# jgrodzki/radix_sort

Hardware: AMD Instinct MI355X
Metric: Gkeys/sec (u64) (higher is better)
Workload: dtype u64

## Files before the change

### radix_sort_amd/csrc/rsx_small_kernel.hpp

```cpp
#pragma once
#include "rsx_device.hpp"

namespace rsx {

struct SmallArgs {
    const void* src;
    void* data;
    uint32_t n;
    uint32_t passes;
    uint32_t rank_atomic;
    uint32_t map_load;
    uint32_t map_store;
    DigitSpec spec[16];
    KeyXform xf;
    const uint32_t* top_tot;
    uint32_t cap;
    uint32_t no_skip;
    uint32_t group_shift;
    uint32_t key_offset, key_bytes;
    uint32_t* hint;
};

struct PassPlan {
    uint32_t first, end;
    uint32_t mask[8];
    uint32_t low[8];
    __device__ __forceinline__ void set_masks(const uint32_t key_offset, const uint32_t key_bytes) {
#pragma unroll
        for (int w = 0; w < 8; ++w) {
            uint32_t m = 0, l = 0;
#pragma unroll
            for (uint32_t b = 0; b < 4; ++b) {
                const uint32_t byte = 4u * (uint32_t)w + b;
                if (byte >= key_offset + first && byte < key_offset + key_bytes) m |= 0xFFu << (8u * b);
                if (byte >= key_offset && byte < key_offset + first) l |= 0xFFu << (8u * b);
            }
            mask[w] = m;
            low[w] = l;
        }
    }
};

#ifndef RSX_MEND_SLACK
#define RSX_MEND_SLACK 6u
#endif
__device__ __forceinline__ uint32_t first_digit_for(const uint32_t m, const uint32_t variable_bits, const uint32_t end) {
    const uint32_t lg = m <= 1u ? 0u : 32u - (uint32_t)__builtin_clz(m - 1u);
    const uint32_t need = 2u * lg > RSX_MEND_SLACK ? 2u * lg - RSX_MEND_SLACK : 0u;
    uint32_t first = variable_bits > need ? (variable_bits - need) >> 3 : 0u;
    if (first + 1u > end) first = end != 0u ? end - 1u : 0u;
    return first;
}

template <int ES>
struct WaveCnt {
    static constexpr bool HALF = false;
    using T = typename std::conditional<HALF, uint16_t, uint32_t>::type;
    static __device__ __forceinline__ void zero(T* my, uint32_t lane) {
        uint32_t* w = reinterpret_cast<uint32_t*>(my);
#pragma unroll
        for (int i = 0; i < (HALF ? 2 : 4); ++i) w[i * WAVE + lane] = 0;
    }
    static __device__ __forceinline__ uint32_t add_rtn(T* my, uint32_t d, uint32_t v) {
        if constexpr (HALF) {
            const uint32_t sh = (d & 1u) * 16u;
            return (atomicAdd(reinterpret_cast<uint32_t*>(my) + (d >> 1), v << sh) >> sh) & 0xFFFFu;
        } else {
            return atomicAdd(&my[d], v);
        }
    }
};
template <int ES, int KPT, int WG>
__host__ __device__ constexpr uint32_t cape() {
    constexpr uint32_t slots = (uint32_t)WG * KPT;
    constexpr uint32_t room = ((163840u - 1024u - (uint32_t)(WG / WAVE) * RADIX * (uint32_t)sizeof(typename WaveCnt<ES>::T) - 64u - 3u * RADIX * 4u) / (uint32_t)ES) & ~3u;
    return slots < room ? slots : room;
}

template <int ES, int KPT, int WG>
__device__ __forceinline__ void local_load(const SmallArgs& a, const Elem<ES>* __restrict__ src, const uint32_t n, Elem<ES> (&e)[KPT]) {
    const uint32_t tid = threadIdx.x, lane = tid & 63u, wave = tid >> 6;
    const uint32_t kp = (n + WG - 1) / WG;
    const uint32_t seg = wave * (WAVE * kp) + lane;
#pragma unroll
    for (int j = 0; j < KPT; ++j) {
        e[j] = Elem<ES>{};
        if ((uint32_t)j < kp) {
            const uint32_t p = seg + (uint32_t)j * WAVE;
            if (p < n) {
                e[j] = src[p];
                if (a.map_load) key_map<ES, false>(e[j], a.xf);
            }
        }
    }
}

template <int ES, int KPT, int WG>
__device__ __forceinline__ void local_passes(const SmallArgs& a, Elem<ES> (&e)[KPT], const uint32_t n, unsigned char* smem,
                                             const uint32_t first = 0, const uint32_t end = ~0u) {
    const uint32_t stop = end == ~0u ? a.passes : end;
    constexpr int NWAVE = WG / WAVE;
    using E = Elem<ES>;
    E* s_elems = reinterpret_cast<E*>(smem);
    using C = WaveCnt<ES>;
    typename C::T* s_cnt = reinterpret_cast<typename C::T*>(smem + (size_t)cape<ES, KPT, WG>() * sizeof(E));
    uint32_t* s_misc = reinterpret_cast<uint32_t*>(s_cnt + NWAVE * RADIX);
    const uint32_t tid = threadIdx.x, lane = tid & 63u, wave = tid >> 6;
    const uint32_t kp = (n + WG - 1) / WG;
    const uint32_t seg = wave * (WAVE * kp) + lane;
    typename C::T* my = s_cnt + wave * RADIX;
    for (uint32_t pass = first; pass < stop; ++pass) {
        const DigitSpec spec = a.spec[pass];
        C::zero(my, lane);
        auto digit_of = [&](int j) -> uint32_t {
            return (seg + (uint32_t)j * WAVE >= n) ? 255u : elem_digit<ES, false>(e[j], spec);
        };
        uint32_t rk[KPT];
#pragma unroll
        for (int j = 0; j < KPT; ++j) {
            rk[j] = 0;
            if ((uint32_t)j < kp) {
                const uint32_t d = digit_of(j);
                if (a.rank_atomic) {
                    rk[j] = C::add_rtn(my, d, 1u);
                } else {
                    const uint64_t m = match_digit(d);
                    const uint32_t below = mbcnt64(m);
                    const uint32_t seen = my[d];
                    if (below == 0) (void)C::add_rtn(my, d, (uint32_t)__popcll(m));
                    rk[j] = seen + below;
                }
            }
        }
        __syncthreads();
        uint32_t tcount = 0, incl = 0;
        if (tid < RADIX) {
#pragma unroll
            for (int w = 0; w < NWAVE; ++w) tcount += s_cnt[w * RADIX + tid];
            incl = wave_incl_scan<true>(tcount);
            if (lane == 63) s_misc[wave] = incl;
        }
        __syncthreads();
        if (tid < RADIX) {
            uint32_t run = incl - tcount;
            for (uint32_t w = 0; w < wave; ++w) run += s_misc[w];
#pragma unroll
            for (int w = 0; w < NWAVE; ++w) {
                const uint32_t c = s_cnt[w * RADIX + tid];
                s_cnt[w * RADIX + tid] = (typename C::T)run;
                run += c;
            }
        }
        __syncthreads();
#pragma unroll
        for (int j = 0; j < KPT; ++j)
            if ((uint32_t)j < kp) {
                if constexpr (cape<ES, KPT, WG>() < (uint32_t)WG * KPT) {
                    if (seg + (uint32_t)j * WAVE < n) s_elems[(uint32_t)my[digit_of(j)] + rk[j]] = e[j];
                } else {
                    s_elems[(uint32_t)my[digit_of(j)] + rk[j]] = e[j];
                }
            }
        __syncthreads();
        if (pass + 1 < stop) {
#pragma unroll
            for (int j = 0; j < KPT; ++j)
                if ((uint32_t)j < kp) e[j] = s_elems[seg + (uint32_t)j * WAVE];
        }
    }
}

template <int ES, int KPT, int WG>
__device__ __forceinline__ void local_store(const SmallArgs& a, Elem<ES>* __restrict__ dst, const uint32_t n, unsigned char* smem) {
    const Elem<ES>* s_elems = reinterpret_cast<const Elem<ES>*>(smem);
    for (uint32_t i = threadIdx.x; i < n; i += WG) {
        Elem<ES> x = s_elems[i];
        if (a.map_store) key_map<ES, true>(x, a.xf);
        dst[i] = x;
    }
}

template <int ES, int KPT, int WG>
__device__ __forceinline__ void local_sort(const SmallArgs& a, const Elem<ES>* __restrict__ src, Elem<ES>* __restrict__ dst,
                                           const uint32_t n, unsigned char* smem) {
    Elem<ES> e[KPT];
    local_load<ES, KPT, WG>(a, src, n, e);
    local_passes<ES, KPT, WG>(a, e, n, smem);
    local_store<ES, KPT, WG>(a, dst, n, smem);
}

template <int ES, int KPT, int WG, typename DigitFn>
__device__ __forceinline__ void stream_pass(const SmallArgs& a, const Elem<ES>* __restrict__ src, Elem<ES>* __restrict__ dst, const uint32_t m,
                                            unsigned char* smem, DigitFn digit, const bool map_back, uint32_t& bin_start, uint32_t& bin_count) {
    constexpr int NWAVE = WG / WAVE;
    constexpr uint32_t CH = cape<ES, KPT, WG>();
    using E = Elem<ES>;
    E* s_elems = reinterpret_cast<E*>(smem);
    using C = WaveCnt<ES>;
    typename C::T* s_cnt = reinterpret_cast<typename C::T*>(smem + (size_t)cape<ES, KPT, WG>() * sizeof(E));
    uint32_t* s_misc = reinterpret_cast<uint32_t*>(s_cnt + NWAVE * RADIX);
    uint32_t* s_gbase = s_misc + NWAVE;
    uint32_t* s_dstart = s_gbase + RADIX;
    uint32_t* s_dcount = s_dstart + RADIX;
    const uint32_t tid = threadIdx.x, lane = tid & 63u, wave = tid >> 6;
    typename C::T* my = s_cnt + wave * RADIX;
    if (tid < RADIX) s_gbase[tid] = 0;
    __syncthreads();
    for (uint32_t i = tid; i < m; i += WG) atomicAdd(&s_gbase[digit(src[i])], 1u);
    __syncthreads();
    if (tid < RADIX) {
        const uint32_t c = s_gbase[tid];
        const uint32_t incl = wave_incl_scan<true>(c);
        if (lane == 63) s_misc[wave] = incl;
        s_dcount[tid] = incl - c;
        bin_count = c;
    }
    __syncthreads();
    if (tid < RADIX) {
        uint32_t b = s_dcount[tid];
        for (uint32_t w = 0; w < wave; ++w) b += s_misc[w];
        s_gbase[tid] = b;
        bin_start = b;
    }
    __syncthreads();
    for (uint32_t c0 = 0; c0 < m; c0 += CH) {
        const uint32_t n = m - c0 < CH ? m - c0 : CH;
        const uint32_t kp = (n + WG - 1) / WG;
        const uint32_t seg = wave * (WAVE * kp) + lane;
        E e[KPT];
#pragma unroll
        for (int j = 0; j < KPT; ++j) {
            e[j] = E{};
            if ((uint32_t)j < kp) {
                const uint32_t p = seg + (uint32_t)j * WAVE;
                if (p < n) e[j] = src[c0 + p];
            }
        }
        C::zero(my, lane);
        auto digit_of = [&](int j) -> uint32_t { return (seg + (uint32_t)j * WAVE >= n) ? 255u : digit(e[j]); };
        uint32_t rk[KPT];
#pragma unroll
        for (int j = 0; j < KPT; ++j) {
            rk[j] = 0;
            if ((uint32_t)j < kp) {
                const uint32_t d = digit_of(j);
                const uint64_t mm = match_digit(d);
                const uint32_t below = mbcnt64(mm);
                const uint32_t seen = my[d];
                if (below == 0) (void)C::add_rtn(my, d, (uint32_t)__popcll(mm));
                rk[j] = seen + below;
            }
        }
        __syncthreads();
        uint32_t tcount = 0, incl = 0;
        if (tid < RADIX) {
#pragma unroll
            for (int w = 0; w < NWAVE; ++w) tcount += s_cnt[w * RADIX + tid];
            incl = wave_incl_scan<true>(tcount);
            if (lane == 63) s_misc[wave] = incl;
        }
        __syncthreads();
        if (tid < RADIX) {
            uint32_t run = incl - tcount;
            for (uint32_t w = 0; w < wave; ++w) run += s_misc[w];
            s_dstart[tid] = run;
            s_dcount[tid] = tid == RADIX - 1 ? tcount - (kp * WG - n) : tcount;
#pragma unroll
            for (int w = 0; w < NWAVE; ++w) {
                const uint32_t c = s_cnt[w * RADIX + tid];
                s_cnt[w * RADIX + tid] = (typename C::T)run;
                run += c;
            }
        }
        __syncthreads();
#pragma unroll
        for (int j = 0; j < KPT; ++j)
            if ((uint32_t)j < kp) {
                if constexpr (cape<ES, KPT, WG>() < (uint32_t)WG * KPT) {
                    if (seg + (uint32_t)j * WAVE < n) s_elems[(uint32_t)my[digit_of(j)] + rk[j]] = e[j];
                } else {
                    s_elems[(uint32_t)my[digit_of(j)] + rk[j]] = e[j];
                }
            }
        __syncthreads();
        for (uint32_t i = tid; i < n; i += WG) {
            E x = s_elems[i];
            const uint32_t d = digit(x);
            const uint32_t pos = s_gbase[d] + (i - s_dstart[d]);
            if (map_back) key_map<ES, true>(x, a.xf);
            dst[pos] = x;
        }
        __syncthreads();
        if (tid < RADIX) s_gbase[tid] += s_dcount[tid];
        __syncthreads();
    }
    __builtin_amdgcn_fence(__ATOMIC_RELEASE, "agent");
    __syncthreads();
    __builtin_amdgcn_fence(__ATOMIC_ACQUIRE, "agent");
}

template <int ES, int KPT, int WG>
__device__ void big_bucket_sort(const SmallArgs& a, Elem<ES>* buf0, Elem<ES>* buf1, const uint32_t m, unsigned char* smem) {
    using E = Elem<ES>;
    E* src = buf0;
    E* dst = buf1;
    for (uint32_t pass = 0; pass < a.passes; ++pass) {
        const DigitSpec spec = a.spec[pass];
        uint32_t bs = 0, bc = 0;
        stream_pass<ES, KPT, WG>(a, src, dst, m, smem, [&](const E& x) { return elem_digit<ES, false>(x, spec); },
                                 pass + 1 == a.passes && a.map_store != 0, bs, bc);
        E* t = src;
        src = dst;
        dst = t;
    }
}

#define RSX_B16_WAVES(WG) ((WG) >= 512 ? 4 : 3)
template <int ES>
__device__ __forceinline__ bool agree(const PassPlan& pp, const Elem<ES>& x, const Elem<ES>& y) {
    uint32_t diff = 0;
#pragma unroll
    for (int w = 0; w < ES / 4; ++w) diff |= (x.w[w] ^ y.w[w]) & pp.mask[w];
    return diff == 0;
}
constexpr uint32_t MEND_LIST = 192;
template <int ES, int KPT, int WG>
__device__ __forceinline__ uint32_t* mend_count(unsigned char* smem) {
    return reinterpret_cast<uint32_t*>(smem + (size_t)cape<ES, KPT, WG>() * sizeof(Elem<ES>));
}
template <int ES, int KPT, int WG>
__device__ __forceinline__ bool local_check(const PassPlan& pp, const uint32_t n, unsigned char* smem, Elem<ES> (&x)[KPT], uint32_t& ties) {
    using E = Elem<ES>;
    const E* s_elems = reinterpret_cast<const E*>(smem);
    ties = 0;
    if (threadIdx.x == 0) *mend_count<ES, KPT, WG>(smem) = 0;
#pragma unroll
    for (int j = 0; j < KPT; ++j) {
        const uint32_t i = (uint32_t)j * WG + threadIdx.x;
        x[j] = E{};
        if (i < n) {
            x[j] = s_elems[i];
            const E p = s_elems[i != 0 ? i - 1 : 0];
            uint32_t diff = 0;
#pragma unroll
            for (int w = 0; w < ES / 4; ++w) diff |= (x[j].w[w] ^ p.w[w]) & pp.mask[w];
            ties |= (diff == 0 && i != 0) ? 1u << j : 0u;
        }
    }
    uint32_t work = 0;
    for (uint32_t t = ties; t != 0; t &= t - 1u) {
        const uint32_t i = (uint32_t)__builtin_ctz(t) * WG + threadIdx.x;
        const E u = s_elems[i], v = s_elems[i - 1];
#pragma unroll
        for (int w = 0; w < ES / 4; ++w) work |= (u.w[w] ^ v.w[w]) & pp.low[w];
    }
    return __syncthreads_or(work != 0 ? 1 : 0) != 0;
}
#ifndef RSX_MEND_INLINE
#define RSX_MEND_INLINE __forceinline__
#endif
template <int ES>
struct MendMasks {
    uint32_t hi[ES / 4], lo[ES / 4];
};
template <int ES>
__device__ RSX_MEND_INLINE uint32_t mend_listed(Elem<ES>* s_elems, uint32_t* s_list, uint32_t* s_flag, const uint32_t n, const uint32_t wg,
                                                          uint32_t ties, const MendMasks<ES> mm) {
    using E = Elem<ES>;
    constexpr uint32_t MAX_RUN = 48;
    auto same = [&](const E& u, const E& v) {
        uint32_t diff = 0;
#pragma unroll
        for (int w = 0; w < ES / 4; ++w) diff |= (u.w[w] ^ v.w[w]) & mm.hi[w];
        return diff == 0;
    };
    auto less = [&](const E& u, const E& v) {
#pragma unroll
        for (int w = ES / 4 - 1; w >= 0; --w) {
            const uint32_t a = u.w[w] & mm.lo[w], b = v.w[w] & mm.lo[w];
            if (a != b) return a < b;
        }
        return false;
    };
    if (threadIdx.x == 0) *s_flag = 0;
    for (uint32_t j = 0; ties != 0; ++j, ties >>= 1) {
        if (!(ties & 1u)) continue;
        const uint32_t i = j * wg + threadIdx.x;
        if (i >= 2 && same(s_elems[i - 1], s_elems[i - 2])) continue;
        const uint32_t k = atomicAdd(&s_list[0], 1u);
        if (k < MEND_LIST) s_list[1 + k] = i - 1;
    }
    __syncthreads();
    const uint32_t heads = s_list[0];
    if (heads > MEND_LIST) return 0u;
    if (threadIdx.x < heads) {
        const uint32_t i = s_list[1 + threadIdx.x];
        uint32_t len = 2;
        while (i + len < n && len <= MAX_RUN && same(s_elems[i + len], s_elems[i])) ++len;
        if (len > MAX_RUN) {
            *s_flag = 1;
        } else {
            for (uint32_t k = 1; k < len; ++k) {
                const E y = s_elems[i + k];
                uint32_t j = k;
                while (j > 0 && less(y, s_elems[i + j - 1])) {
                    s_elems[i + j] = s_elems[i + j - 1];
                    --j;
                }
                s_elems[i + j] = y;
            }
        }
    }
    __syncthreads();
    return *s_flag == 0 ? 1u : 0u;
}
template <int ES, int KPT, int WG>
__device__ __forceinline__ bool local_mend_listed(const uint32_t n, unsigned char* smem, const PassPlan& pp, uint32_t* s_flag, const uint32_t ties) {
    static_assert((WG / WAVE) * RADIX >= MEND_LIST + 1, "the list lives in the wave counters");
    MendMasks<ES> mm;
#pragma unroll
    for (int w = 0; w < ES / 4; ++w) {
        mm.hi[w] = pp.mask[w];
        mm.lo[w] = pp.low[w];
    }
    return mend_listed<ES>(reinterpret_cast<Elem<ES>*>(smem), mend_count<ES, KPT, WG>(smem), s_flag, n, (uint32_t)WG, ties, mm) != 0;
}
template <int ES, int KPT, int WG>
__device__ __forceinline__ void local_store_regs(const SmallArgs& a, Elem<ES>* __restrict__ dst, const uint32_t n, Elem<ES> (&x)[KPT]) {
#pragma unroll
    for (int j = 0; j < KPT; ++j) {
        const uint32_t i = (uint32_t)j * WG + threadIdx.x;
        if (i < n) {
            if (a.map_store) key_map<ES, true>(x[j], a.xf);
            dst[i] = x[j];
        }
    }
}

template <int ES, int KPT, int WG>
__device__ __forceinline__ bool local_finish(const SmallArgs& a, Elem<ES>* __restrict__ dst, const uint32_t n, unsigned char* smem, const PassPlan& pp,
                                             uint32_t* s_flag) {
    Elem<ES> x[KPT];
    uint32_t ties;
    if (!local_check<ES, KPT, WG>(pp, n, smem, x, ties)) {
        local_store_regs<ES, KPT, WG>(a, dst, n, x);
        return true;
    }
    if (!local_mend_listed<ES, KPT, WG>(n, smem, pp, s_flag, ties)) return false;
    local_store<ES, KPT, WG>(a, dst, n, smem);
    return true;
}

template <int ES, int KPT, int WG>
__device__ __forceinline__ void local_sort_skip(const SmallArgs& a, const Elem<ES>* __restrict__ src, Elem<ES>* __restrict__ dst, const uint32_t n,
                                                unsigned char* smem, PassPlan& pp, uint32_t* s_flag) {
    using E = Elem<ES>;
    E e[KPT];
    local_load<ES, KPT, WG>(a, src, n, e);
    local_passes<ES, KPT, WG>(a, e, n, smem, pp.first, pp.end);
    if (pp.first == 0) {
        local_store<ES, KPT, WG>(a, dst, n, smem);
    } else if (!local_finish<ES, KPT, WG>(a, dst, n, smem, pp, s_flag)) {
        pp.first = 0;
        const uint32_t kp = (n + WG - 1) / WG, seg = (threadIdx.x >> 6) * (WAVE * kp) + (threadIdx.x & 63u);
#pragma unroll
        for (int j = 0; j < KPT; ++j)
            if ((uint32_t)j < kp) e[j] = reinterpret_cast<const E*>(smem)[seg + (uint32_t)j * WAVE];
        __syncthreads();
        local_passes<ES, KPT, WG>(a, e, n, smem, 0, pp.end);
        local_store<ES, KPT, WG>(a, dst, n, smem);
    }
}

template <int ES, int KPT>
__global__ __launch_bounds__(512) void rsx_small_sort_kernel(const SmallArgs a) {
    extern __shared__ __attribute__((aligned(16))) unsigned char smem[];
    local_sort<ES, KPT, 512>(a, static_cast<const Elem<ES>*>(a.src), static_cast<Elem<ES>*>(a.data), a.n, smem);
}

template <int ES, int KPT, int WG>
__global__ __launch_bounds__(WG) void rsx_bucket_sort_kernel(const SmallArgs a) {
    extern __shared__ __attribute__((aligned(16))) unsigned char smem[];
    uint64_t* s_red = reinterpret_cast<uint64_t*>(smem);
    const uint32_t tid = threadIdx.x, v = blockIdx.x;
    uint64_t c = 0;
    if (tid < RADIX) {
        c = a.top_tot[tid];
        if (tid == v) s_red[4] = c;
        if (v == 0) {
            uint64_t big = c;
#pragma unroll
            for (int o = 32; o > 0; o >>= 1) {
                const uint64_t y = __shfl_xor(big, o);
                big = y > big ? y : big;
            }
            if ((tid & 63u) == 0u) s_red[5 + (tid >> 6)] = big;
        }
        uint64_t below = tid < v ? c : 0ull;
#pragma unroll
        for (int o = 32; o > 0; o >>= 1) below += __shfl_xor(below, o);
        if ((tid & 63u) == 0u) s_red[tid >> 6] = below;
    }
    __syncthreads();
    const uint64_t start = s_red[0] + s_red[1] + s_red[2] + s_red[3];
    const uint64_t count = s_red[4];
    if (v == 0 && tid == 0) {
        uint64_t big = s_red[5];
        for (int w = 1; w < 4; ++w) big = s_red[5 + w] > big ? s_red[5 + w] : big;
        __hip_atomic_store(a.hint, big <= (uint64_t)a.cap / 4 ? 1u : big <= (uint64_t)a.cap ? 3u : 2u, __ATOMIC_RELAXED, __HIP_MEMORY_SCOPE_SYSTEM);
    }
    __syncthreads();
    if (count == 0) return;
    if (count > (uint64_t)cape<ES, KPT, WG>()) {
        big_bucket_sort<ES, KPT, WG>(a, const_cast<Elem<ES>*>(static_cast<const Elem<ES>*>(a.src)) + start,
                                     static_cast<Elem<ES>*>(a.data) + start, (uint32_t)count, smem);
        return;
    }
    if constexpr (ES < 8) {
        local_sort<ES, KPT, WG>(a, static_cast<const Elem<ES>*>(a.src) + start, static_cast<Elem<ES>*>(a.data) + start, (uint32_t)count, smem);
    } else {
        PassPlan pp;
        pp.end = a.passes;
        pp.first = a.no_skip ? 0u : first_digit_for((uint32_t)count, 8u * a.passes, a.passes);
        pp.set_masks(a.key_offset, a.key_bytes);
        uint32_t* s_flag = reinterpret_cast<uint32_t*>(reinterpret_cast<typename WaveCnt<ES>::T*>(smem + (size_t)cape<ES, KPT, WG>() * sizeof(Elem<ES>)) + (WG / WAVE) * RADIX) + (WG / WAVE);
        local_sort_skip<ES, KPT, WG>(a, static_cast<const Elem<ES>*>(a.src) + start, static_cast<Elem<ES>*>(a.data) + start, (uint32_t)count, smem, pp,
                                     s_flag);
    }
}

template <int ES, int KPT, int WG>
__global__ __launch_bounds__(WG, RSX_B16_WAVES(WG)) void rsx_bucket16_kernel(const SmallArgs a, const uint64_t* __restrict__ starts, void* scratch,
                                                                         const WidePlan* __restrict__ plan, Gate gate) {
    extern __shared__ __attribute__((aligned(16))) unsigned char smem[];
    if (!gate_open(gate)) return;
    using E = Elem<ES>;
    constexpr int NWAVE = WG / WAVE;
    uint32_t* s_flag = reinterpret_cast<uint32_t*>(reinterpret_cast<typename WaveCnt<ES>::T*>(smem + (size_t)cape<ES, KPT, WG>() * sizeof(E)) + NWAVE * RADIX) + NWAVE;
    const uint32_t gs = a.group_shift != 0 ? plan->group_shift : 0;
    const bool medium = (plan->verdict & VERDICT_MEDIUM) != 0;
    PassPlan pp;
    pp.end = gs == 0 ? plan->pass_end : plan->group_end;
    if (pp.end == 0) {
        if (a.map_store) {
            const uint64_t n = starts[65536];
            E* data = static_cast<E*>(a.data);
            for (uint64_t i = (uint64_t)blockIdx.x * WG + threadIdx.x; i < n; i += (uint64_t)gridDim.x * WG) {
                E x = data[i];
                key_map<ES, true>(x, a.xf);
                data[i] = x;
            }
        }
        return;
    }
    const uint32_t b_lo = plan->window_top - 15u;
    const uint32_t end_sub = pp.end;
    if (gs != 0) pp.end = (b_lo + gs + 7u) / 8u;
    {
        const uint64_t big = (uint64_t)plan->scan_max << gs;
        const uint32_t m = big < (uint64_t)cape<ES, KPT, WG>() ? (uint32_t)big : cape<ES, KPT, WG>();
        pp.first = a.no_skip ? 0u : first_digit_for(m, b_lo + gs, pp.end);
    }
    pp.set_masks(a.key_offset, a.key_bytes);
    for (uint32_t g = blockIdx.x; g < (65536u >> gs); g += gridDim.x) {
        const uint32_t b0 = g << gs;
        const uint64_t gstart = starts[b0];
        const uint64_t gcount = starts[b0 + (1u << gs)] - gstart;
        if (gcount == 0) continue;
        const bool whole = gs == 0 || gcount <= (uint64_t)cape<ES, KPT, WG>();
        const uint32_t nsub = whole ? 1u : 1u << gs;
        for (uint32_t sub = 0; sub < nsub; ++sub) {
            uint64_t start = gstart, count = gcount;
            if (!whole) {
                start = starts[b0 + sub];
                count = starts[b0 + sub + 1] - start;
            }
            if (count != 0) {
                E* bucket = static_cast<E*>(a.data) + start;
                if (count <= (uint64_t)cape<ES, KPT, WG>()) {
                    const uint32_t first = pp.first, end = pp.end;
                    if (!whole) {
                        pp.first = 0;
                        pp.end = end_sub;
                    }
                    local_sort_skip<ES, KPT, WG>(a, bucket, bucket, (uint32_t)count, smem, pp, s_flag);
                    if (!whole) {
                        pp.first = first;
                        pp.end = end;
                    }
                } else if (!medium) {
                    big_bucket_sort<ES, KPT, WG>(a, bucket, static_cast<E*>(scratch) + start, (uint32_t)count, smem);
                }
            }
            __syncthreads();
        }
    }
}

template <int ES, int KPT, int WG>
__global__ __launch_bounds__(WG, RSX_B16_WAVES(WG)) void rsx_bucket16_medium_kernel(const SmallArgs a, const uint64_t* __restrict__ starts, void* scratch,
                                                                                const WidePlan* __restrict__ plan, uint32_t cap256, uint32_t cap512,
                                                                                uint32_t cap1024, Gate gate) {
    extern __shared__ __attribute__((aligned(16))) unsigned char smem[];
    __shared__ uint32_t s_part[2];
    if (!gate_open(gate)) return;
    using E = Elem<ES>;
    constexpr int NWAVE = WG / WAVE;
    constexpr uint32_t CAPE = cape<ES, KPT, WG>();
    uint32_t* s_flag = reinterpret_cast<uint32_t*>(reinterpret_cast<typename WaveCnt<ES>::T*>(smem + (size_t)CAPE * sizeof(E)) + NWAVE * RADIX) + NWAVE;
    const uint32_t tid = threadIdx.x;
    const uint32_t form = plan->verdict & VERDICT_FORM_MASK;
    const uint64_t handled = form == VERDICT_WG256 ? cap256 : form == VERDICT_WG1024 ? cap1024 : cap512;
    const uint32_t end = plan->pass_end;
    if (end == 0) return;
    const uint32_t b_lo = plan->window_top - 15u;
    for (uint32_t b = blockIdx.x; b < 65536u; b += gridDim.x) {
        const uint64_t start = starts[b];
        const uint64_t count = starts[b + 1] - start;
        if (count <= handled) continue;
        E* bucket = static_cast<E*>(a.data) + start;
        E* scr = static_cast<E*>(scratch) + start;
        uint32_t k = 0;
        while (k < 8u && (count >> k) > (uint64_t)CAPE * 6u / 10u) ++k;
        if (k > b_lo) k = b_lo;
        const bool split = !(k == 0 || (count >> k) > (uint64_t)CAPE || count > 0xFFFFFFFFull);
        uint32_t kmask = 0, part_start = 0, part_count = (uint32_t)count;
        PassPlan pp;
        pp.end = end;
        pp.first = 0;
        if (split) {
            DigitSpec sp{};
            const uint32_t ebit = 8u * a.key_offset + b_lo - k;
            sp.word = ebit >> 5;
            sp.shift = ebit & 31u;
            kmask = (1u << k) - 1u;
            part_start = part_count = 0;
            const uint32_t km = kmask;
            stream_pass<ES, KPT, WG>(a, bucket, scr, (uint32_t)count, smem, [&](const E& x) { return elem_digit_any<ES>(x, sp) & km; }, false, part_start,
                                     part_count);
            const uint32_t keep = plan->keep + (k >= 4u ? 1u : 0u);
            pp.first = (end > keep && !a.no_skip) ? end - keep : 0;
            pp.set_masks(a.key_offset, a.key_bytes);
        }
        for (uint32_t j = 0; j <= kmask; ++j) {
            __syncthreads();
            if (tid == j) {
                s_part[0] = part_start;
                s_part[1] = part_count;
            }
            __syncthreads();
            const uint32_t off = s_part[0], cnt = s_part[1];
            if (cnt == 0) continue;
            if (split && cnt <= CAPE) {
                local_sort_skip<ES, KPT, WG>(a, scr + off, bucket + off, cnt, smem, pp, s_flag);
            } else {
                if (split) {
                    for (uint32_t i = tid; i < cnt; i += WG) bucket[off + i] = scr[off + i];
                    __builtin_amdgcn_fence(__ATOMIC_RELEASE, "agent");
                    __syncthreads();
                    __builtin_amdgcn_fence(__ATOMIC_ACQUIRE, "agent");
                }
                big_bucket_sort<ES, KPT, WG>(a, bucket + off, scr + off, cnt, smem);
            }
        }
        __syncthreads();
    }
}

}
```

Measured before the change: 67.75.

## Replace listed mend with per-thread inline insertion mend and looser digit-skip margin

```diff
diff --git a/radix_sort_amd/csrc/rsx_small_kernel.hpp b/radix_sort_amd/csrc/rsx_small_kernel.hpp
--- a/radix_sort_amd/csrc/rsx_small_kernel.hpp
+++ b/radix_sort_amd/csrc/rsx_small_kernel.hpp
@@ -41,12 +41,12 @@
     }
 };
 
-#ifndef RSX_MEND_SLACK
-#define RSX_MEND_SLACK 6u
+#ifndef RSX_MEND_MARGIN
+#define RSX_MEND_MARGIN 1u
 #endif
 __device__ __forceinline__ uint32_t first_digit_for(const uint32_t m, const uint32_t variable_bits, const uint32_t end) {
     const uint32_t lg = m <= 1u ? 0u : 32u - (uint32_t)__builtin_clz(m - 1u);
-    const uint32_t need = 2u * lg > RSX_MEND_SLACK ? 2u * lg - RSX_MEND_SLACK : 0u;
+    const uint32_t need = lg + RSX_MEND_MARGIN;
     uint32_t first = variable_bits > need ? (variable_bits - need) >> 3 : 0u;
     if (first + 1u > end) first = end != 0u ? end - 1u : 0u;
     return first;
@@ -323,17 +323,13 @@
     for (int w = 0; w < ES / 4; ++w) diff |= (x.w[w] ^ y.w[w]) & pp.mask[w];
     return diff == 0;
 }
-constexpr uint32_t MEND_LIST = 192;
-template <int ES, int KPT, int WG>
-__device__ __forceinline__ uint32_t* mend_count(unsigned char* smem) {
-    return reinterpret_cast<uint32_t*>(smem + (size_t)cape<ES, KPT, WG>() * sizeof(Elem<ES>));
-}
-template <int ES, int KPT, int WG>
-__device__ __forceinline__ bool local_check(const PassPlan& pp, const uint32_t n, unsigned char* smem, Elem<ES> (&x)[KPT], uint32_t& ties) {
+template <int ES, int KPT, int WG>
+__device__ __forceinline__ bool local_check(const PassPlan& pp, const uint32_t n, unsigned char* smem, Elem<ES> (&x)[KPT], uint32_t& ties,
+                                             uint32_t* s_flag) {
     using E = Elem<ES>;
     const E* s_elems = reinterpret_cast<const E*>(smem);
     ties = 0;
-    if (threadIdx.x == 0) *mend_count<ES, KPT, WG>(smem) = 0;
+    if (threadIdx.x == 0) *s_flag = 0;
 #pragma unroll
     for (int j = 0; j < KPT; ++j) {
         const uint32_t i = (uint32_t)j * WG + threadIdx.x;
@@ -356,74 +352,53 @@
     }
     return __syncthreads_or(work != 0 ? 1 : 0) != 0;
 }
-#ifndef RSX_MEND_INLINE
-#define RSX_MEND_INLINE __forceinline__
+#ifndef RSX_MEND_RUN
+#define RSX_MEND_RUN 16u
 #endif
-template <int ES>
-struct MendMasks {
-    uint32_t hi[ES / 4], lo[ES / 4];
-};
-template <int ES>
-__device__ RSX_MEND_INLINE uint32_t mend_listed(Elem<ES>* s_elems, uint32_t* s_list, uint32_t* s_flag, const uint32_t n, const uint32_t wg,
-                                                          uint32_t ties, const MendMasks<ES> mm) {
-    using E = Elem<ES>;
-    constexpr uint32_t MAX_RUN = 48;
-    auto same = [&](const E& u, const E& v) {
-        uint32_t diff = 0;
-#pragma unroll
-        for (int w = 0; w < ES / 4; ++w) diff |= (u.w[w] ^ v.w[w]) & mm.hi[w];
-        return diff == 0;
-    };
+template <int ES, int KPT, int WG>
+__device__ __forceinline__ bool local_mend(const PassPlan& pp, const uint32_t n, unsigned char* smem, uint32_t* s_flag, uint32_t ties) {
+    using E = Elem<ES>;
+    E* s_elems = reinterpret_cast<E*>(smem);
     auto less = [&](const E& u, const E& v) {
 #pragma unroll
         for (int w = ES / 4 - 1; w >= 0; --w) {
-            const uint32_t a = u.w[w] & mm.lo[w], b = v.w[w] & mm.lo[w];
+            const uint32_t a = u.w[w] & pp.low[w], b = v.w[w] & pp.low[w];
             if (a != b) return a < b;
         }
         return false;
     };
-    if (threadIdx.x == 0) *s_flag = 0;
-    for (uint32_t j = 0; ties != 0; ++j, ties >>= 1) {
-        if (!(ties & 1u)) continue;
-        const uint32_t i = j * wg + threadIdx.x;
-        if (i >= 2 && same(s_elems[i - 1], s_elems[i - 2])) continue;
-        const uint32_t k = atomicAdd(&s_list[0], 1u);
-        if (k < MEND_LIST) s_list[1 + k] = i - 1;
-    }
-    __syncthreads();
-    const uint32_t heads = s_list[0];
-    if (heads > MEND_LIST) return 0u;
-    if (threadIdx.x < heads) {
-        const uint32_t i = s_list[1 + threadIdx.x];
-        uint32_t len = 2;
-        while (i + len < n && len <= MAX_RUN && same(s_elems[i + len], s_elems[i])) ++len;
-        if (len > MAX_RUN) {
-            *s_flag = 1;
-        } else {
-            for (uint32_t k = 1; k < len; ++k) {
-                const E y = s_elems[i + k];
-                uint32_t j = k;
-                while (j > 0 && less(y, s_elems[i + j - 1])) {
-                    s_elems[i + j] = s_elems[i + j - 1];
+    for (; ties != 0; ties &= ties - 1u) {
+        const uint32_t h = (uint32_t)__builtin_ctz(ties) * WG + threadIdx.x - 1u;
+        const E hd = s_elems[h];
+        if (h != 0 && agree<ES>(pp, hd, s_elems[h - 1])) continue;
+        E top = hd;
+        E y = s_elems[h + 1];
+        uint32_t k = 1;
+        while (true) {
+            if (k == RSX_MEND_RUN) {
+                *s_flag = 1;
+                break;
+            }
+            if (less(y, top)) {
+                s_elems[h + k] = top;
+                uint32_t j = k - 1;
+                while (j > 0) {
+                    const E z = s_elems[h + j - 1];
+                    if (!less(y, z)) break;
+                    s_elems[h + j] = z;
                     --j;
                 }
-                s_elems[i + j] = y;
-            }
-        }
-    }
-    __syncthreads();
-    return *s_flag == 0 ? 1u : 0u;
-}
-template <int ES, int KPT, int WG>
-__device__ __forceinline__ bool local_mend_listed(const uint32_t n, unsigned char* smem, const PassPlan& pp, uint32_t* s_flag, const uint32_t ties) {
-    static_assert((WG / WAVE) * RADIX >= MEND_LIST + 1, "the list lives in the wave counters");
-    MendMasks<ES> mm;
-#pragma unroll
-    for (int w = 0; w < ES / 4; ++w) {
-        mm.hi[w] = pp.mask[w];
-        mm.lo[w] = pp.low[w];
-    }
-    return mend_listed<ES>(reinterpret_cast<Elem<ES>*>(smem), mend_count<ES, KPT, WG>(smem), s_flag, n, (uint32_t)WG, ties, mm) != 0;
+                s_elems[h + j] = y;
+            } else {
+                top = y;
+            }
+            if (++k + h >= n) break;
+            y = s_elems[h + k];
+            if (!agree<ES>(pp, y, hd)) break;
+        }
+    }
+    __syncthreads();
+    return *s_flag == 0;
 }
 template <int ES, int KPT, int WG>
 __device__ __forceinline__ void local_store_regs(const SmallArgs& a, Elem<ES>* __restrict__ dst, const uint32_t n, Elem<ES> (&x)[KPT]) {
@@ -442,11 +417,11 @@
                                              uint32_t* s_flag) {
     Elem<ES> x[KPT];
     uint32_t ties;
-    if (!local_check<ES, KPT, WG>(pp, n, smem, x, ties)) {
+    if (!local_check<ES, KPT, WG>(pp, n, smem, x, ties, s_flag)) {
         local_store_regs<ES, KPT, WG>(a, dst, n, x);
         return true;
     }
-    if (!local_mend_listed<ES, KPT, WG>(n, smem, pp, s_flag, ties)) return false;
+    if (!local_mend<ES, KPT, WG>(pp, n, smem, s_flag, ties)) return false;
     local_store<ES, KPT, WG>(a, dst, n, smem);
     return true;
 }
```

Result: no change. 68.15 (median of 6 runs) (+0.6%).
